# jcyk/gtos

Hardware: AMD Instinct MI355X
Metric: graphs/sec training step (100-node AMR, batch 64) (higher is better)
Workload: dtype bf16

## Files before the change

gtos_amd/build.py:

```python
import os
import subprocess
import sys

CSRC = os.path.join(os.path.dirname(os.path.abspath(__file__)), "csrc")
LIB = os.path.join(CSRC, "libgtos_hip.so")
SOURCES = ["gemm.hip", "rel_attn.hip", "rowops.hip", "gru_step.hip", "copy_nll.hip", "tokenenc.hip", "pathtrie_dev.hip", "relbatch_dev.hip", "relindex_dev.hip", "beam.hip", "sample.hip", "copy_ls.hip", "copy_eval.hip"]
EXACT_FP = {"relbatch_dev.hip", "beam.hip", "sample.hip"}
HIPCC = os.environ.get("HIPCC", "/opt/rocm/bin/hipcc")
FLAGS = ["--offload-arch=gfx950", "-O3", "-std=c++17", "-fPIC", "-ffast-math", "-fno-finite-math-only"]


def _stale(target, deps):
    if not os.path.exists(target):
        return True
    t = os.path.getmtime(target)
    return any(os.path.getmtime(d) > t for d in deps)


def _deps(obj, fallback):
    dfile = obj[:-2] + ".d"
    root = os.path.dirname(os.path.dirname(CSRC))
    try:
        words = open(dfile).read().replace("\\\n", " ").split()
    except OSError:
        return fallback
    deps = [w for w in words[1:] if w.endswith((".h", ".hpp")) and os.path.abspath(w).startswith(root) and os.path.exists(w)]
    return deps or fallback


HOST_SRCS = [os.path.join(os.path.dirname(CSRC), "csrc_host", f) for f in ("relbatch.cpp", "pathtrie.cpp", "relindex.cpp")]
HOST_LIB = os.path.join(os.path.dirname(CSRC), "csrc_host", "libgtos_host.so")
CXX = os.environ.get("CXX", "g++")


def build_host(force=False, verbose=True):
    hdr = os.path.join(os.path.dirname(os.path.dirname(CSRC)), "include", "gtos_host.h")
    shared = [os.path.join(CSRC, h) for h in ("relbatch_kernels.h", "relindex_kernels.h", "trie_kernels.h")]
    if force or _stale(HOST_LIB, HOST_SRCS + [hdr] + shared):
        cmd = [CXX, "-O3", "-std=c++17", "-shared", "-fPIC", "-pthread"] + HOST_SRCS + ["-o", HOST_LIB]
        if verbose:
            print(" ".join(cmd), flush=True)
        subprocess.check_call(cmd)
    return HOST_LIB


def build(force=False, verbose=True):
    build_host(force, verbose)
    own_hdr = {"pathtrie_dev.hip": "trie_kernels.h", "relbatch_dev.hip": "relbatch_kernels.h",
               "relindex_dev.hip": "relindex_kernels.h", "beam.hip": "beam_kernels.h slot_kernels.h slot_device.h",
               "sample.hip": "sample_kernels.h slot_kernels.h slot_device.h", "copy_ls.hip": "copy_ls_kernels.h",
               "copy_nll.hip": "copy_row.h", "copy_eval.hip": "copy_eval_kernels.h"}
    objs = []
    for src in SOURCES:
        s = os.path.join(CSRC, src)
        o = os.path.join(CSRC, src.replace(".hip", ".o"))
        objs.append(o)
        if force or _stale(o, [s] + _deps(o, [os.path.join(CSRC, h) for h in own_hdr.get(src, "common.h").split()])):
            flags = [f for f in FLAGS if f not in ("-ffast-math", "-fno-finite-math-only")] + ["-ffp-contract=off"] if src in EXACT_FP else FLAGS
            cmd = [HIPCC] + flags + ["-MMD", "-MF", o[:-2] + ".d", "-c", s, "-o", o]
            if verbose:
                print(" ".join(cmd), flush=True)
            subprocess.check_call(cmd)
    if force or _stale(LIB, objs):
        cmd = [HIPCC, "--offload-arch=gfx950", "-shared", "-fPIC"] + objs + ["-o", LIB]
        if verbose:
            print(" ".join(cmd), flush=True)
        subprocess.check_call(cmd)
    return LIB


if __name__ == "__main__":
    build(force="--force" in sys.argv)
    print(LIB)
```

gtos_amd/csrc/common.h:

```cpp
#pragma once
#include <hip/hip_runtime.h>
#include <stdint.h>

#define GTOS_F32 0
#define GTOS_BF16 1

typedef uint16_t bf16_t;
typedef __attribute__((ext_vector_type(8))) __bf16 bf16x8_t;
typedef __attribute__((ext_vector_type(8))) short s16x8_t;
typedef __attribute__((ext_vector_type(4))) float f32x4_t;

typedef __attribute__((ext_vector_type(4))) uint32_t U128;

__device__ __forceinline__ float bf2f(bf16_t v) { return __uint_as_float(((uint32_t)v) << 16); }
typedef __attribute__((ext_vector_type(2))) __bf16 bf16x2_hw_t;
typedef __attribute__((ext_vector_type(2))) float f32x2_hw_t;
__device__ __forceinline__ bf16_t f2bf(float f) { return __builtin_bit_cast(bf16_t, static_cast<__bf16>(f)); }
__device__ __forceinline__ float lo_bf(uint32_t w) { return __uint_as_float(w << 16); }
__device__ __forceinline__ float hi_bf(uint32_t w) { return __uint_as_float(w & 0xffff0000u); }
__device__ __forceinline__ uint32_t pack_bf(float a, float b) {
    const f32x2_hw_t v = {a, b};
    return __builtin_bit_cast(uint32_t, __builtin_convertvector(v, bf16x2_hw_t));
}

template <typename T> struct Vec8;
template <> struct Vec8<float> {
    static __device__ __forceinline__ void load(const float* p, float (&v)[8]) {
        const float4 a = *reinterpret_cast<const float4*>(p), b = *reinterpret_cast<const float4*>(p + 4);
        v[0] = a.x; v[1] = a.y; v[2] = a.z; v[3] = a.w; v[4] = b.x; v[5] = b.y; v[6] = b.z; v[7] = b.w;
    }
    static __device__ __forceinline__ void store(float* p, const float (&v)[8]) {
        *reinterpret_cast<float4*>(p) = make_float4(v[0], v[1], v[2], v[3]);
        *reinterpret_cast<float4*>(p + 4) = make_float4(v[4], v[5], v[6], v[7]);
    }
};
template <> struct Vec8<bf16_t> {
    static __device__ __forceinline__ void load(const bf16_t* p, float (&v)[8]) {
        const uint4 a = *reinterpret_cast<const uint4*>(p);
        v[0] = lo_bf(a.x); v[1] = hi_bf(a.x); v[2] = lo_bf(a.y); v[3] = hi_bf(a.y);
        v[4] = lo_bf(a.z); v[5] = hi_bf(a.z); v[6] = lo_bf(a.w); v[7] = hi_bf(a.w);
    }
    static __device__ __forceinline__ void store(bf16_t* p, const float (&v)[8]) {
        *reinterpret_cast<uint4*>(p) = make_uint4(pack_bf(v[0], v[1]), pack_bf(v[2], v[3]),
                                                  pack_bf(v[4], v[5]), pack_bf(v[6], v[7]));
    }
};

template <typename T> __device__ __forceinline__ float to_f(T v);
template <> __device__ __forceinline__ float to_f<float>(float v) { return v; }
template <> __device__ __forceinline__ float to_f<bf16_t>(bf16_t v) { return bf2f(v); }
template <typename T> __device__ __forceinline__ T from_f(float v);
template <> __device__ __forceinline__ float from_f<float>(float v) { return v; }
template <> __device__ __forceinline__ bf16_t from_f<bf16_t>(float v) { return f2bf(v); }

__device__ __forceinline__ uint32_t mix32(uint32_t h) {
    h ^= h >> 16; h *= 0x7feb352dU; h ^= h >> 15; h *= 0x846ca68bU; h ^= h >> 16;
    return h;
}
__device__ __forceinline__ float rand01(uint64_t seed, uint64_t idx) {
    uint32_t h = mix32((uint32_t)idx ^ (uint32_t)seed);
    h = mix32(h + (uint32_t)(idx >> 32) * 0x9E3779B9U + (uint32_t)(seed >> 32));
    return (float)(h >> 8) * (1.0f / 16777216.0f);
}
__device__ __forceinline__ bool drop_keep(uint64_t seed, uint64_t idx, float p) { return rand01(seed, idx) >= p; }

static __device__ const unsigned long long* g_seed_epoch = nullptr;
__device__ __forceinline__ uint64_t live_seed(uint64_t seed) {
    const unsigned long long* p = g_seed_epoch;
    return p ? seed + (uint64_t)(*p) * 0x9E3779B97F4A7C15ull : seed;
}
#define GTOS_SEED_EPOCH_SETTER(tu)                                                                                   \
    extern "C" __attribute__((visibility("hidden"))) int gtosi_##tu##_set_seed_epoch(const void* p) {               \
        return (int)hipMemcpyToSymbol(HIP_SYMBOL(g_seed_epoch), &p, sizeof(p));                                      \
    }
extern "C" __attribute__((visibility("hidden"))) int gtosi_gemm_set_seed_epoch(const void* p);
extern "C" __attribute__((visibility("hidden"))) int gtosi_rel_attn_set_seed_epoch(const void* p);
extern "C" __attribute__((visibility("hidden"))) int gtosi_rowops_set_seed_epoch(const void* p);
extern "C" __attribute__((visibility("hidden"))) int gtosi_gru_step_set_seed_epoch(const void* p);
extern "C" __attribute__((visibility("hidden"))) int gtosi_tokenenc_set_seed_epoch(const void* p);

__device__ __forceinline__ float wave_sum(float v) {
#pragma unroll
    for (int o = 32; o > 0; o >>= 1) v += __shfl_xor(v, o);
    return v;
}
__device__ __forceinline__ float wave_max(float v) {
#pragma unroll
    for (int o = 32; o > 0; o >>= 1) v = fmaxf(v, __shfl_xor(v, o));
    return v;
}

#define GTOS_CHECK_LAUNCH() do { hipError_t e_ = hipGetLastError(); if (e_ != hipSuccess) return (int)e_; } while (0)
```

gtos_amd/csrc/rel_attn.hip:

```cpp
#include "common.h"
#include <cstdlib>
#include <type_traits>

namespace {

template <typename T> struct Raw8;
template <> struct Raw8<bf16_t> {
    uint4 a;
    __device__ __forceinline__ void load(const bf16_t* p) { a = *reinterpret_cast<const uint4*>(p); }
    __device__ __forceinline__ void zero() { a = make_uint4(0, 0, 0, 0); }
    __device__ __forceinline__ void get(float (&v)[8]) const {
        v[0] = lo_bf(a.x); v[1] = hi_bf(a.x); v[2] = lo_bf(a.y); v[3] = hi_bf(a.y);
        v[4] = lo_bf(a.z); v[5] = hi_bf(a.z); v[6] = lo_bf(a.w); v[7] = hi_bf(a.w);
    }
};
template <> struct Raw8<float> {
    float4 a, b;
    __device__ __forceinline__ void load(const float* p) {
        a = *reinterpret_cast<const float4*>(p); b = *reinterpret_cast<const float4*>(p + 4);
    }
    __device__ __forceinline__ void zero() { a = make_float4(0, 0, 0, 0); b = a; }
    __device__ __forceinline__ void get(float (&v)[8]) const {
        v[0] = a.x; v[1] = a.y; v[2] = a.z; v[3] = a.w; v[4] = b.x; v[5] = b.y; v[6] = b.z; v[7] = b.w;
    }
};

#ifndef GTOS_ATTN_U
#define GTOS_ATTN_U 1
#endif
template <typename T> struct Unroll { static constexpr int U = GTOS_ATTN_U; };
template <> struct Unroll<float> { static constexpr int U = 1; };

struct AttnArgs {
    const void *q, *k, *v; int64_t ldq, ldk, ldv;
    const void* rel;
    const int* idx_q;
    const int* idx_k;
    const uint8_t* key_pad;
    const uint8_t* attn_mask;
    void* o; int64_t ldo;
    float* lse;
    float* w;
    const void* d_o; int64_t lddo;
    const float* dw;
    void *dq, *dk, *dv; int64_t lddq, lddk, lddv;
    int64_t ld_drel;
    void* d_rel;
    float* pd;
    float* gs;
    int T, S, B, H, d, mode;
    int hd, nhs, lr;
    float scale, p_drop; uint64_t seed;
};
// ... 494 lines not shown
#pragma unroll
                for (int e = 0; e < 8; ++e) { r1[e] = fmaf(gsum, RB[e], da[e]); r2[e] = fmaf(gsum, RA[e], db[e]); }
                Vec8<T>::store(out, r1);
                Vec8<T>::store(out + d, r2);
            }
        }
        m1 = m2; l1 = l2; m2 = m3;
    }
}

template <typename K> int dispatch_lh(int lh, K&& f) {
    switch (lh) {
        case 1: return f(std::integral_constant<int, 1>());
        case 2: return f(std::integral_constant<int, 2>());
        case 4: return f(std::integral_constant<int, 4>());
        case 8: return f(std::integral_constant<int, 8>());
        case 16: return f(std::integral_constant<int, 16>());
        case 32: return f(std::integral_constant<int, 32>());
        case 64: return f(std::integral_constant<int, 64>());
    }
    return -11;
}

struct Geo { int LH, nhs, lr, slices; bool generic; };
int pow2ceil(int x) { int p = 1; while (p < x) p <<= 1; return p; }
int geometry(int d, int H, Geo& g) {
    if (H <= 0 || d <= 0 || d % H) return -10;
    const int hd = d / H;
    if (hd % 8 || hd > 512) return -10;
    g.generic = !(d <= 512 && (d & (d - 1)) == 0 && (hd & (hd - 1)) == 0);
    if (!g.generic) { g.LH = hd / 8; g.nhs = H; g.lr = d / 8; g.slices = 1; return 0; }
    g.LH = pow2ceil(hd / 8);
    int nhs = 64 / g.LH;
    const int hp = pow2ceil(H);
    if (nhs > hp) nhs = hp;
    g.nhs = nhs; g.lr = nhs * g.LH; g.slices = (H + nhs - 1) / nhs;
    return 0;
}
int check_shape(int d, int H) { Geo g; return geometry(d, H, g); }

int nblocks(int rows, int B) { return rows * B; }

}

static int fill_args(AttnArgs& a, Geo& g, int T_, int S, int B, int H, int d, int mode, float scale, float p_drop, uint64_t seed) {
    a.T = T_; a.S = S; a.B = B; a.H = H; a.d = d; a.mode = mode; a.scale = scale; a.p_drop = p_drop; a.seed = seed;
    if (mode != 0 && T_ != S) return -12;
    const int rc = geometry(d, H, g);
    if (rc) return rc;
    a.hd = d / H; a.nhs = g.nhs; a.lr = g.lr;
    return 0;
}

extern "C" int gtos_rel_attn_fwd(int dtype, int mode, int T_, int S, int B, int H, int d,
                                 const void* q, int64_t ldq, const void* k, int64_t ldk, const void* v, int64_t ldv,
                                 const void* rel, const int* idx_q, const uint8_t* key_pad, const uint8_t* attn_mask,
                                 float scale, float p_drop, uint64_t seed,
                                 void* o, int64_t ldo, float* lse, float* w, void* stream) {
    AttnArgs a = {};
    Geo geo;
    int rc = fill_args(a, geo, T_, S, B, H, d, mode, scale, p_drop, seed);
    if (rc) return rc;
    a.q = q; a.k = k; a.v = v; a.ldq = ldq; a.ldk = ldk; a.ldv = ldv; a.rel = rel; a.idx_q = idx_q;
    a.key_pad = key_pad; a.attn_mask = attn_mask; a.o = o; a.ldo = ldo; a.lse = lse; a.w = w;
    hipStream_t s = static_cast<hipStream_t>(stream);
    const dim3 grid(nblocks(T_, B), geo.slices);
    return dispatch_lh(geo.LH, [&](auto lh) {
        constexpr int LH = decltype(lh)::value;
        if (geo.generic) {
            if (dtype == GTOS_BF16) hipLaunchKernelGGL((rel_attn_fwd_kernel<bf16_t, LH, true>), grid, dim3(256), 0, s, a);
            else hipLaunchKernelGGL((rel_attn_fwd_kernel<float, LH, true>), grid, dim3(256), 0, s, a);
        } else {
            if (dtype == GTOS_BF16) hipLaunchKernelGGL((rel_attn_fwd_kernel<bf16_t, LH, false>), grid, dim3(256), 0, s, a);
            else hipLaunchKernelGGL((rel_attn_fwd_kernel<float, LH, false>), grid, dim3(256), 0, s, a);
        }
        GTOS_CHECK_LAUNCH();
        return 0;
    });
}

extern "C" int gtos_rel_attn_bwd(int dtype, int mode, int T_, int S, int B, int H, int d,
                                 const void* q, int64_t ldq, const void* k, int64_t ldk, const void* v, int64_t ldv,
                                 const void* rel, const int* idx_q, const int* idx_k,
                                 const uint8_t* key_pad, const uint8_t* attn_mask,
                                 float scale, float p_drop, uint64_t seed,
                                 const void* o, int64_t ldo, const float* lse, const float* w,
                                 const void* d_o, int64_t lddo, const float* dw,
                                 void* dq, int64_t lddq, void* dk, int64_t lddk, void* dv, int64_t lddv,
                                 void* d_rel, int64_t ld_drel, float* pd, float* gs, void* stream) {
    AttnArgs a = {};
    Geo geo;
    int rc = fill_args(a, geo, T_, S, B, H, d, mode, scale, p_drop, seed);
    if (rc) return rc;
    a.q = q; a.k = k; a.v = v; a.ldq = ldq; a.ldk = ldk; a.ldv = ldv; a.rel = rel; a.idx_q = idx_q; a.idx_k = idx_k;
    a.key_pad = key_pad; a.attn_mask = attn_mask; a.o = const_cast<void*>(o); a.ldo = ldo;
    a.lse = const_cast<float*>(lse); a.w = const_cast<float*>(w); a.d_o = d_o; a.lddo = lddo; a.dw = dw;
    a.dq = dq; a.dk = dk; a.dv = dv; a.lddq = lddq; a.lddk = lddk; a.lddv = lddv; a.d_rel = d_rel; a.ld_drel = ld_drel; a.pd = pd; a.gs = gs;
    if (mode == 2 && d_rel && (ld_drel < 2 * d || ld_drel % 8)) return -14;
    if (dw && !w) return -13;
    hipStream_t s = static_cast<hipStream_t>(stream);
    const dim3 gq(nblocks(T_, B), geo.slices), gk(nblocks(S, B), geo.slices);
    return dispatch_lh(geo.LH, [&](auto lh) {
        constexpr int LH = decltype(lh)::value;
#define GTOS_BWD(TT, GG) do { hipLaunchKernelGGL((rel_attn_bwd_q_kernel<TT, LH, GG>), gq, dim3(256), 0, s, a); \
                              hipLaunchKernelGGL((rel_attn_bwd_kv_kernel<TT, LH, GG>), gk, dim3(256), 0, s, a); } while (0)
        if (geo.generic) { if (dtype == GTOS_BF16) GTOS_BWD(bf16_t, true); else GTOS_BWD(float, true); }
        else { if (dtype == GTOS_BF16) GTOS_BWD(bf16_t, false); else GTOS_BWD(float, false); }
#undef GTOS_BWD
        GTOS_CHECK_LAUNCH();
        return 0;
    });
}

extern "C" int gtos_rel_attn_bwd_bank(int dtype, int n, int B, int H, int d,
                                      const void* q, int64_t ldq, const void* k, int64_t ldk,
                                      const void* bank, const float* gs,
                                      const int* pair_sorted, const int* chunk_type, const int* chunk_start,
                                      const int* chunk_count, const int* chunk_slot, const int* xcd_off, int nchunks,
                                      void* d_bank, int64_t ld_dbank, float* heavy, void* stream) {
    Geo geo;
    int rc = geometry(d, H, geo);
    if (rc) return rc;
    if (ld_dbank < 2 * d || ld_dbank % 8) return -14;
    if (nchunks <= 0) return 0;
    BankArgs a;
    a.q = q; a.k = k; a.ldq = ldq; a.ldk = ldk; a.bank = bank; a.gs = gs; a.pair_sorted = pair_sorted;
    a.chunk_type = chunk_type; a.chunk_start = chunk_start; a.chunk_count = chunk_count; a.chunk_slot = chunk_slot;
    a.d_bank = d_bank; a.ld_dbank = ld_dbank; a.heavy = heavy; a.nchunks = nchunks; a.T = n; a.S = n; a.B = B; a.H = H; a.d = d;
    a.xcd_off = xcd_off;
    a.hd = d / H; a.nhs = geo.nhs; a.lr = geo.lr;
    hipStream_t s = static_cast<hipStream_t>(stream);
    int grid = (nchunks + 3) / 4; if (grid > 4096) grid = 4096;
    if (xcd_off) grid = (grid + 7) / 8 * 8;
    const dim3 g2(grid, geo.slices);
    return dispatch_lh(geo.LH, [&](auto lh) {
        constexpr int LH = decltype(lh)::value;
        if (geo.generic) {
            if (dtype == GTOS_BF16) hipLaunchKernelGGL((rel_attn_bwd_bank_kernel<bf16_t, LH, true, 4>), g2, dim3(256), 0, s, a);
            else hipLaunchKernelGGL((rel_attn_bwd_bank_kernel<float, LH, true, 4>), g2, dim3(256), 0, s, a);
        } else {
            if (dtype == GTOS_BF16) hipLaunchKernelGGL((rel_attn_bwd_bank_kernel<bf16_t, LH, false, 2>), g2, dim3(256), 0, s, a);
            else hipLaunchKernelGGL((rel_attn_bwd_bank_kernel<float, LH, false, 4>), g2, dim3(256), 0, s, a);
        }
        GTOS_CHECK_LAUNCH();
        return 0;
    });
}

GTOS_SEED_EPOCH_SETTER(rel_attn)
```

gtos_amd/csrc/rowops.hip:

```cpp
#include "common.h"

namespace {

constexpr int LN_MAXC = 2;

template <typename TX, typename TR, typename TY>
__global__ __launch_bounds__(256) void ln_fwd_kernel(int rows, int d, const TX* __restrict__ x, const TR* __restrict__ r,
                                                     float p_drop, uint64_t seed, const float* __restrict__ gamma,
                                                     const float* __restrict__ beta, float eps, TY* __restrict__ y, bf16_t* __restrict__ y2,
                                                     float* __restrict__ mean, float* __restrict__ rstd) {
    if (p_drop > 0.f) seed = live_seed(seed);
    const int lane = threadIdx.x & 63;
    const int row = blockIdx.x * 4 + (threadIdx.x >> 6);
    if (row >= rows) return;
    const float ks = p_drop > 0.f ? 1.f / (1.f - p_drop) : 1.f;
    float z[LN_MAXC][8];
    float s = 0.f;
#pragma unroll
    for (int cI = 0; cI < LN_MAXC; ++cI) {
        const int c = (cI * 64 + lane) * 8;
#pragma unroll
        for (int e = 0; e < 8; ++e) z[cI][e] = 0.f;
        if (c < d) {
            Vec8<TX>::load(x + (int64_t)row * d + c, z[cI]);
// ... 1060 lines not shown
extern "C" int gtos_adam_step(int64_t n, float* p, const float* g, float* m, float* v, float lr, float beta1, float beta2,
                              float eps, float weight_decay, float gscale, const float* sqnorm, float max_norm,
                              void* bf16_mirror, void* stream) {
    if (n <= 0) return 0;
    hipStream_t s = static_cast<hipStream_t>(stream);
    hipLaunchKernelGGL(adam_kernel, dim3(grid_for(n, 256 * 4)), dim3(256), 0, s, n, p, g, m, v, lr, beta1, beta2, eps, weight_decay,
                       gscale, sqnorm, max_norm, (bf16_t*)bf16_mirror, (const float*)nullptr);
    GTOS_CHECK_LAUNCH();
    return 0;
}

extern "C" int gtos_adam_step_ctl(int64_t n, float* p, const float* g, float* m, float* v, const float* ctl, float beta1, float beta2,
                                  float eps, float weight_decay, float gscale, const float* sqnorm, float max_norm,
                                  void* bf16_mirror, void* stream) {
    if (n <= 0) return 0;
    if (!ctl) return -23;
    hipStream_t s = static_cast<hipStream_t>(stream);
    hipLaunchKernelGGL(adam_kernel, dim3(grid_for(n, 256 * 4)), dim3(256), 0, s, n, p, g, m, v, 0.f, beta1, beta2, eps, weight_decay,
                       gscale, sqnorm, max_norm, (bf16_t*)bf16_mirror, ctl);
    GTOS_CHECK_LAUNCH();
    return 0;
}

extern "C" int gtos_step_control(int phase, const float* loss, double* state, float* flag, int warmup_steps, int embed_dim,
                                 float* ctl, void* stream) {
    if ((phase != 0 && phase != 1) || !loss || !state || !flag || !ctl || warmup_steps < 1 || embed_dim < 1) return -23;
    hipLaunchKernelGGL(step_control_kernel, dim3(1), dim3(64), 0, static_cast<hipStream_t>(stream), phase, loss, state, flag,
                       (double)warmup_steps, (double)embed_dim, ctl);
    GTOS_CHECK_LAUNCH();
    return 0;
}

extern "C" int gtos_cast_f32_to_bf16(int64_t n, const float* src, void* dst, void* stream) {
    if (n <= 0) return 0;
    hipStream_t s = static_cast<hipStream_t>(stream);
    hipLaunchKernelGGL(cast_bf16_kernel, dim3(grid_for(n, 256 * 4)), dim3(256), 0, s, n, src, (bf16_t*)dst);
    GTOS_CHECK_LAUNCH();
    return 0;
}

extern "C" int gtos_transpose_batch_bf16(int n_mat, const int64_t* desc, const int* tile_start, int total_tiles, const void* src,
                                         void* dst, void* stream) {
    if (n_mat <= 0 || total_tiles <= 0) return 0;
    if (!desc || !tile_start || !src || !dst) return -23;
    hipLaunchKernelGGL(transpose_batch_kernel, dim3((unsigned)total_tiles), dim3(256), 0, static_cast<hipStream_t>(stream), n_mat, desc,
                       tile_start, (const bf16_t*)src, (bf16_t*)dst);
    GTOS_CHECK_LAUNCH();
    return 0;
}

extern "C" int gtos_set_seed_epoch(const void* epoch) {
    int rc = gtosi_gemm_set_seed_epoch(epoch);
    if (!rc) rc = gtosi_rel_attn_set_seed_epoch(epoch);
    if (!rc) rc = gtosi_rowops_set_seed_epoch(epoch);
    if (!rc) rc = gtosi_gru_step_set_seed_epoch(epoch);
    if (!rc) rc = gtosi_tokenenc_set_seed_epoch(epoch);
    return rc;
}

extern "C" int gtos_abi_version(void) { return 25; }

GTOS_SEED_EPOCH_SETTER(rowops)
```

gtos_amd/ops.py:

```python
import contextlib
import os

import torch

from . import _lib
from ._lib import call, dt, ptr, require_cuda, stream

_seed_state = [0x5DEECE66D]

PROFILE = None
PROFILE_DETAIL = False
GEMM_PROFILE = None


class _Timed:

    def __init__(self, name, detail=False, units=0):
        self.name, self.units = name, units
        self.on = PROFILE is not None and (PROFILE_DETAIL or not detail)

    def __enter__(self):
        if self.on:
            self.s = torch.cuda.Event(enable_timing=True)
            self.e = torch.cuda.Event(enable_timing=True)
# ... 625 lines not shown
        starts = bounds[:-1]
        nch = torch.clamp((counts + self.CHUNK - 1) // self.CHUNK, min=1)
        ctype = torch.repeat_interleave(torch.arange(R, device=flat.device), nch)
        first = torch.cumsum(nch, 0) - nch
        local = torch.arange(ctype.numel(), device=flat.device) - first[ctype]
        heavy_types = torch.nonzero(nch > 1).flatten()
        slot_of_type = torch.full((R,), -1, dtype=torch.int64, device=flat.device)
        slot_of_type[heavy_types] = torch.arange(heavy_types.numel(), device=flat.device)
        self.pair_sorted = order.to(torch.int32)
        c_type = ctype.to(torch.int32)
        c_start = (starts[ctype] + local * self.CHUNK).to(torch.int32)
        c_count = torch.clamp(counts[ctype] - local * self.CHUNK, min=0, max=self.CHUNK).to(torch.int32)
        c_slot = slot_of_type[ctype].to(torch.int32)
        first = self.pair_sorted[c_start.clamp(max=flat.numel() - 1).long()]
        gb = first % B
        xcd = (gb // (B // 8)) if B % 8 == 0 else (gb % 8)
        xs, perm = torch.sort(xcd.to(torch.int32), stable=True)
        self.xcd_off = torch.searchsorted(xs, torch.arange(9, device=flat.device, dtype=torch.int32)).to(torch.int32)
        self.chunk_type, self.chunk_start = c_type[perm], c_start[perm]
        self.chunk_count, self.chunk_slot = c_count[perm], c_slot[perm]
        self.heavy_types = heavy_types.to(torch.int32)
        self.nchunks = int(ctype.numel())

    def prefetch_projections(self, attns):
        self._proj = {}
        if not (PROJ_SIDE and self.bank.is_cuda and side_ok(self.bank.device) and torch.is_grad_enabled()):
            return
        dev = self.bank.device
        main, side = torch.cuda.current_stream(dev), side_stream(dev)
        if any(m.compute_dtype != self.bank.dtype for m in attns):
            return
        if sum(self.bank.shape[0] * m.relation_in_proj.weight.shape[0] for m in attns) * self.bank.element_size() > PROJ_SIDE_MAX_BYTES:
            return
        side.wait_stream(main)
        self.bank.record_stream(side)
        with torch.cuda.stream(side):
            for m in attns:
                y = linear(self.bank, m.relation_in_proj.weight, group=self.grad_group)
                ev = torch.cuda.Event()
                ev.record(side)
                self._proj[id(m)] = (y, ev)

    def take_projection(self, attn):
        hit = self._proj.pop(id(attn), None)
        if hit is None:
            return None
        y, ev = hit
        main = torch.cuda.current_stream(y.device)
        main.wait_event(ev)
        y.record_stream(main)
        return y


class RelAttnFn(torch.autograd.Function):

    @staticmethod
    def forward(ctx, qsrc, kvsrc, rel, fact, offs, d, H, scale, key_pad, attn_mask, p_drop, need_w):
        require_cuda(qsrc, kvsrc, rel)
        q_off, k_off, v_off = offs
        kv = qsrc if kvsrc is None else kvsrc
        assert qsrc.is_contiguous() and kv.is_contiguous()
        T_, B, Cq = qsrc.shape
        S, _, Ckv = kv.shape
        mode = 0 if rel is None else (2 if fact is not None else 1)
        if mode == 1:
            assert rel.is_contiguous() and tuple(rel.shape) == (S, T_, B, 2 * d)
        o = torch.empty((T_, B, d), dtype=qsrc.dtype, device=qsrc.device)
        lse = torch.empty((T_, B, H), dtype=torch.float32, device=qsrc.device)
        w = torch.empty((T_, S, B, H), dtype=torch.float32, device=qsrc.device) if need_w else None
        seed = next_seed() if p_drop > 0 else 0
        es = qsrc.element_size()
        with _Timed("rel_attn_fwd_mode%d" % mode):
            call("gtos_rel_attn_fwd", dt(qsrc), mode, T_, S, B, H, d,
                 qsrc.data_ptr() + q_off * es, Cq, kv.data_ptr() + k_off * es, Ckv, kv.data_ptr() + v_off * es, Ckv,
                 ptr(rel), ptr(fact.idx_q) if fact is not None else None, ptr(key_pad), ptr(attn_mask),
                 float(scale), float(p_drop), seed, ptr(o), d, ptr(lse), ptr(w), stream())
        src = getattr(rel, "_gtos_proj_src", None) if (mode == 2 and PROJ_RECOMPUTE) else None
        ctx.save_for_backward(qsrc, kvsrc, rel if src is None else None, o, lse, w, key_pad, attn_mask)
        ctx.cfg = (fact, offs, d, H, scale, p_drop, seed, mode)
        ctx.proj_src = src
        return o, w

    @staticmethod
    def backward(ctx, d_o, d_w):
        qsrc, kvsrc, rel, o, lse, w, key_pad, attn_mask = ctx.saved_tensors
        fact, (q_off, k_off, v_off), d, H, scale, p_drop, seed, mode = ctx.cfg
        if ctx.proj_src is not None:
            bank_, w_ = ctx.proj_src
            rel = gemm(bank_, w_, trans_b=True)
        kv = qsrc if kvsrc is None else kvsrc
        T_, B, Cq = qsrc.shape
        S, _, Ckv = kv.shape
        d_o = d_o.contiguous()
        if d_w is not None:
            d_w = d_w.contiguous().float()
        full_q = (Cq == d) if kvsrc is not None else (Cq == 3 * d)
        dqsrc = (torch.empty_like if full_q else torch.zeros_like)(qsrc)
        dkv = dqsrc if kvsrc is None else (torch.empty_like if Ckv == 2 * d else torch.zeros_like)(kvsrc)
        if mode == 1:
            d_rel = torch.empty_like(rel)
        elif mode == 2:
            d_rel = fact.grad_group.grad_slice(rel) if ctx.needs_input_grad[2] else None
            if d_rel is None:
                d_rel = torch.empty_like(rel)
        else:
            d_rel = None
        ldr = d_rel.stride(0) if mode == 2 else 0
        pd = torch.empty((T_, S, B, H), dtype=torch.float32, device=qsrc.device)
        gs = torch.empty_like(pd)
        es = qsrc.element_size()
        with _Timed("rel_attn_bwd_q+kv_mode%d" % mode, detail=True):
            call("gtos_rel_attn_bwd", dt(qsrc), mode, T_, S, B, H, d,
                 qsrc.data_ptr() + q_off * es, Cq, kv.data_ptr() + k_off * es, Ckv, kv.data_ptr() + v_off * es, Ckv,
                 ptr(rel), ptr(fact.idx_q) if fact is not None else None, ptr(fact.idx_k) if fact is not None else None,
                 ptr(key_pad), ptr(attn_mask), float(scale), float(p_drop), seed,
                 ptr(o), d, ptr(lse), ptr(w), ptr(d_o), d, ptr(d_w),
                 dqsrc.data_ptr() + q_off * es, Cq, dkv.data_ptr() + k_off * es, Ckv, dkv.data_ptr() + v_off * es, Ckv,
                 ptr(d_rel), ldr, ptr(pd), ptr(gs), stream())
        if mode == 2:
            nh = int(fact.heavy_types.numel())
            heavy = torch.zeros((max(nh, 1), 2 * d), dtype=torch.float32, device=rel.device)
            with _Timed("rel_attn_bwd_bank", detail=True):
                call("gtos_rel_attn_bwd_bank", dt(qsrc), T_, B, H, d,
                     qsrc.data_ptr() + q_off * es, Cq, kv.data_ptr() + k_off * es, Ckv,
                     ptr(rel), ptr(gs), ptr(fact.pair_sorted), ptr(fact.chunk_type), ptr(fact.chunk_start),
                     ptr(fact.chunk_count), ptr(fact.chunk_slot), ptr(fact.xcd_off), fact.nchunks, ptr(d_rel), ldr, ptr(heavy), stream())
            if nh and d_rel.dtype == torch.bfloat16:
                call("gtos_segment_sum_finish", nh, ptr(fact.heavy_types), ptr(heavy), 2 * d, ptr(d_rel), ldr, stream())
            elif nh:
                d_rel[fact.heavy_types.long()] = heavy[:nh].to(d_rel.dtype)
        return dqsrc, (dkv if kvsrc is not None else None), d_rel, None, None, None, None, None, None, None, None, None


def attention_core(qsrc, kvsrc, offs, d, H, scale, rel=None, fact=None, key_pad=None, attn_mask=None,
                   p_drop=0.0, need_weights=False):
    return RelAttnFn.apply(qsrc, kvsrc, rel, fact, offs, d, H, scale, _u8(key_pad), _u8(attn_mask),
                           float(p_drop), need_weights)


def factored_eval_relation(bank, relation):
    n, n2, B, K = relation.shape
    tuples, inv = torch.unique(relation.reshape(-1, K), dim=0, return_inverse=True)
    bank_c = relation_gather_mean(bank, tuples, zero_row0=True)
    return FactoredRelation(bank_c, inv.view(n, n2, B))


def relation_gather_mean(bank, idx, zero_row0):
    require_cuda(bank, idx)
    K = idx.shape[-1] if zero_row0 else 1
    lead = idx.shape[:-1] if zero_row0 else idx.shape
    P = idx.numel() // K
    bank = bank.contiguous()
    out = torch.empty((P, bank.shape[1]), dtype=bank.dtype, device=bank.device)
    call("gtos_relation_gather_mean", dt(bank), P, K, bank.shape[1], ptr(bank), ptr(idx.contiguous()), int(zero_row0),
         ptr(out), stream())
    return out.view(*lead, bank.shape[1])


def embed_bwd_workspace(n, V, dim_pad, device):
    if V * dim_pad * 4 > 60 * 1024 or n <= 8 * 512:
        return None
    return torch.empty((min(2048, (n + 511) // 512), V * dim_pad), dtype=torch.float32, device=device)

# ... 370 lines not shown
```

Baseline: 852.1.

## Add MFMA flash-style tiled attention kernels for plain bf16 attention mode

Adds a new tiled attention forward and backward path, used for mode 0 (no relation bias) bf16 attention when head dims are 32/64/128. It stages K/V tiles in shared memory and computes scores and outputs with MFMA bf16 instructions and an online softmax, with a hi/lo split of the probabilities to keep precision. The backward pass runs dK/dV and dQ blocks in one fused launch and no longer allocates the full T×S×B×H fp32 pd/gs scratch tensors. Risks include numeric differences from the old path, and it only applies to mode 0 calls with aligned pointers.

```diff
diff --git a/gtos_amd/build.py b/gtos_amd/build.py
--- a/gtos_amd/build.py
+++ b/gtos_amd/build.py
@@ -4,7 +4,7 @@
 
 CSRC = os.path.join(os.path.dirname(os.path.abspath(__file__)), "csrc")
 LIB = os.path.join(CSRC, "libgtos_hip.so")
-SOURCES = ["gemm.hip", "rel_attn.hip", "rowops.hip", "gru_step.hip", "copy_nll.hip", "tokenenc.hip", "pathtrie_dev.hip", "relbatch_dev.hip", "relindex_dev.hip", "beam.hip", "sample.hip", "copy_ls.hip", "copy_eval.hip"]
+SOURCES = ["gemm.hip", "rel_attn.hip", "attn_tile.hip", "rowops.hip", "gru_step.hip", "copy_nll.hip", "tokenenc.hip", "pathtrie_dev.hip", "relbatch_dev.hip", "relindex_dev.hip", "beam.hip", "sample.hip", "copy_ls.hip", "copy_eval.hip"]
 EXACT_FP = {"relbatch_dev.hip", "beam.hip", "sample.hip"}
 HIPCC = os.environ.get("HIPCC", "/opt/rocm/bin/hipcc")
 FLAGS = ["--offload-arch=gfx950", "-O3", "-std=c++17", "-fPIC", "-ffast-math", "-fno-finite-math-only"]
@@ -49,7 +49,8 @@
     own_hdr = {"pathtrie_dev.hip": "trie_kernels.h", "relbatch_dev.hip": "relbatch_kernels.h",
                "relindex_dev.hip": "relindex_kernels.h", "beam.hip": "beam_kernels.h slot_kernels.h slot_device.h",
                "sample.hip": "sample_kernels.h slot_kernels.h slot_device.h", "copy_ls.hip": "copy_ls_kernels.h",
-               "copy_nll.hip": "copy_row.h", "copy_eval.hip": "copy_eval_kernels.h"}
+               "copy_nll.hip": "copy_row.h", "rel_attn.hip": "common.h attn_tile.h", "attn_tile.hip": "common.h attn_tile.h",
+               "copy_eval.hip": "copy_eval_kernels.h"}
     objs = []
     for src in SOURCES:
         s = os.path.join(CSRC, src)
diff --git a/gtos_amd/csrc/attn_tile.h b/gtos_amd/csrc/attn_tile.h
--- /dev/null
+++ b/gtos_amd/csrc/attn_tile.h
@@ -0,0 +1,20 @@
+#pragma once
+#include <stdint.h>
+
+struct AttnTileArgs {
+    const void *q, *k, *v; int64_t ldq, ldk, ldv;
+    const uint8_t* key_pad;
+    const uint8_t* attn_mask;
+    void* o; int64_t ldo;
+    float* lse;
+    float* w;
+    const void* d_o; int64_t lddo;
+    const float* dw;
+    void *dq, *dk, *dv; int64_t lddq, lddk, lddv;
+    int T, S, B, H, d;
+    float scale, p_drop; uint64_t seed;
+};
+
+bool gtosi_attn_tile_covers(int T, int S, int B, int H, int d, const AttnTileArgs& a, bool backward);
+int gtosi_attn_tile_fwd(const AttnTileArgs& a, void* stream);
+int gtosi_attn_tile_bwd(const AttnTileArgs& a, void* stream);
diff --git a/gtos_amd/csrc/attn_tile.hip b/gtos_amd/csrc/attn_tile.hip
--- /dev/null
+++ b/gtos_amd/csrc/attn_tile.hip
@@ -0,0 +1,422 @@
+#include "common.h"
+#include "attn_tile.h"
+#include <cstdlib>
+#include <type_traits>
+
+namespace {
+
+constexpr int OWN = 64;
+
+template <int HD> struct Cfg {
+    static constexpr int NT = HD == 128 ? 32 : 64;
+    static constexpr int RS = HD + 8;
+    static constexpr int CH = HD / 8;
+    static constexpr int KC = HD / 32;
+    static constexpr int CB = HD / 16;
+    static constexpr int NB = NT / 32;
+    static constexpr int DS = NT + 4;
+};
+
+__device__ __forceinline__ void map_block(int B, int H, int& b, int& h, int& tile) {
+    const int blk = blockIdx.x;
+    int rest;
+    if ((B & 7) == 0) { const int x = blk & 7, w = blk >> 3, gpx = B >> 3; b = x * gpx + (w % gpx); rest = w / gpx; }
+    else { b = blk % B; rest = blk / B; }
+    h = rest % H; tile = rest / H;
+}
+
+__device__ __forceinline__ f32x4_t mfma(bf16x8_t a, bf16x8_t b, f32x4_t c) {
+    return __builtin_amdgcn_mfma_f32_16x16x32_bf16(a, b, c, 0, 0, 0);
+}
+
+template <int HD, bool RM, bool TR>
+__device__ __forceinline__ void stage(const bf16_t* __restrict__ base, int64_t rstride, int r0, int nrows, bf16_t* rm, bf16_t* tr) {
+    using C = Cfg<HD>;
+    constexpr int IT = C::NT * C::CH / 256;
+    uint4 v[IT];
+#pragma unroll
+    for (int it = 0; it < IT; ++it) {
+        const int idx = it * 256 + threadIdx.x, y = idx / C::CH, c = idx % C::CH;
+        v[it] = make_uint4(0, 0, 0, 0);
+        if (r0 + y < nrows) v[it] = *reinterpret_cast<const uint4*>(base + (int64_t)(r0 + y) * rstride + c * 8);
+    }
+#pragma unroll
+    for (int it = 0; it < IT; ++it) {
+        const int idx = it * 256 + threadIdx.x, y = idx / C::CH, c = idx % C::CH;
+        if (RM) *reinterpret_cast<uint4*>(rm + y * C::RS + c * 8) = v[it];
+        if (TR) {
+            const int yc = (((y >> 3) ^ (c & (C::NT / 8 - 1))) << 3) | (y & 7);
+            const uint32_t ww[4] = {v[it].x, v[it].y, v[it].z, v[it].w};
+#pragma unroll
+            for (int e = 0; e < 8; ++e) tr[(c * 8 + e) * C::NT + yc] = (bf16_t)(ww[e >> 1] >> ((e & 1) * 16));
+        }
+    }
+}
+
+template <int HD> __device__ __forceinline__ bf16x8_t frag_rows(const bf16_t* rm, int kb, int t, int kc, int lane) {
+    const int r = lane & 15, row = kb * 32 + (r >> 2) * 8 + t * 4 + (r & 3);
+    return *reinterpret_cast<const bf16x8_t*>(rm + row * Cfg<HD>::RS + kc * 32 + (lane >> 4) * 8);
+}
+template <int HD> __device__ __forceinline__ bf16x8_t frag_tr(const bf16_t* tr, int cb, int kb, int lane) {
+    constexpr int NT = Cfg<HD>::NT;
+    const int cc = cb * 16 + (lane & 15), chunk = (kb * 4 + (lane >> 4)) ^ ((cc >> 3) & (NT / 8 - 1));
+    return *reinterpret_cast<const bf16x8_t*>(tr + cc * NT + chunk * 8);
+}
+template <int HD> __device__ __forceinline__ void load_own(const bf16_t* __restrict__ base, int64_t rstride, int x, bool valid, int lane,
+                                                            bf16x8_t (&f)[Cfg<HD>::KC]) {
+#pragma unroll
+    for (int kc = 0; kc < Cfg<HD>::KC; ++kc) {
+        U128 v = {0, 0, 0, 0};
+        if (valid) v = *reinterpret_cast<const U128*>(base + (int64_t)x * rstride + kc * 32 + (lane >> 4) * 8);
+        f[kc] = __builtin_bit_cast(bf16x8_t, v);
+    }
+}
+__device__ __forceinline__ void split8(const float (&p)[8], bf16x8_t& hi, bf16x8_t& lo) {
+    uint32_t hw[4], lw[4];
+#pragma unroll
+    for (int e = 0; e < 4; ++e) {
+        hw[e] = pack_bf(p[2 * e], p[2 * e + 1]);
+        lw[e] = pack_bf(p[2 * e] - lo_bf(hw[e]), p[2 * e + 1] - hi_bf(hw[e]));
+    }
+    const U128 a = {hw[0], hw[1], hw[2], hw[3]}, b = {lw[0], lw[1], lw[2], lw[3]};
+    hi = __builtin_bit_cast(bf16x8_t, a); lo = __builtin_bit_cast(bf16x8_t, b);
+}
+__device__ __forceinline__ void store4(bf16_t* p, const f32x4_t& v, float s) {
+    *reinterpret_cast<uint2*>(p) = make_uint2(pack_bf(v[0] * s, v[1] * s), pack_bf(v[2] * s, v[3] * s));
+}
+
+template <int HD, bool KM>
+__device__ __forceinline__ void fill_dead(const AttnTileArgs& a, int b, int x0, int y0, unsigned char* sdead) {
+    using C = Cfg<HD>;
+#pragma unroll
+    for (int it = 0; it < OWN * C::NT / 256; ++it) {
+        const int idx = it * 256 + threadIdx.x, xo = idx / C::NT, ys = idx % C::NT;
+        const int i = KM ? y0 + ys : x0 + xo, j = KM ? x0 + xo : y0 + ys;
+        const int ic = min(i, a.T - 1), jc = min(j, a.S - 1);
+        const unsigned char kp = a.key_pad ? a.key_pad[(int64_t)jc * a.B + b] : 0;
+        const unsigned char am = a.attn_mask ? a.attn_mask[(int64_t)ic * a.S + jc] : 0;
+        sdead[xo * C::DS + ys] = (i >= a.T || j >= a.S || kp != 0 || am != 0) ? 1 : 0;
+    }
+}
+
+template <int HD>
+__global__ __launch_bounds__(256) void attn_tile_fwd_kernel(AttnTileArgs a) {
+    using C = Cfg<HD>;
+    if (a.p_drop > 0.f) a.seed = live_seed(a.seed);
+    __shared__ __attribute__((aligned(16))) bf16_t sK[C::NT * C::RS];
+    __shared__ __attribute__((aligned(16))) bf16_t sVt[HD * C::NT];
+    __shared__ __attribute__((aligned(16))) unsigned char sdead[OWN * C::DS];
+    int b, h, qt;
+    map_block(a.B, a.H, b, h, qt);
+    const int lane = threadIdx.x & 63, wv = threadIdx.x >> 6, n = lane & 15, g = lane >> 4;
+    const int i0 = qt * OWN, xo = wv * 16 + n, i = i0 + xo;
+    const bool iv = i < a.T;
+    const int64_t hb = (int64_t)h * HD;
+    const bf16_t* qb = static_cast<const bf16_t*>(a.q) + (int64_t)b * a.ldq + hb;
+    const bf16_t* kb_ = static_cast<const bf16_t*>(a.k) + (int64_t)b * a.ldk + hb;
+    const bf16_t* vb = static_cast<const bf16_t*>(a.v) + (int64_t)b * a.ldv + hb;
+    const int64_t rsq = (int64_t)a.B * a.ldq, rsk = (int64_t)a.B * a.ldk, rsv = (int64_t)a.B * a.ldv;
+    const float keep_scale = a.p_drop > 0.f ? 1.f / (1.f - a.p_drop) : 1.f;
+
+    bf16x8_t xq[C::KC];
+    load_own<HD>(qb, rsq, i, iv, lane, xq);
+    float m = -INFINITY, l = 0.f;
+    f32x4_t oacc[C::CB];
+#pragma unroll
+    for (int cb = 0; cb < C::CB; ++cb) oacc[cb] = f32x4_t{0.f, 0.f, 0.f, 0.f};
+
+    for (int j0 = 0; j0 < a.S; j0 += C::NT) {
+        __syncthreads();
+        stage<HD, true, false>(kb_, rsk, j0, a.S, sK, nullptr);
+        stage<HD, false, true>(vb, rsv, j0, a.S, nullptr, sVt);
+        fill_dead<HD, false>(a, b, i0, j0, sdead);
+        __syncthreads();
+        float s[C::NB][8];
+        float mt = -INFINITY;
+#pragma unroll
+        for (int kb = 0; kb < C::NB; ++kb) {
+#pragma unroll
+            for (int t = 0; t < 2; ++t) {
+                f32x4_t part[C::KC];
+#pragma unroll
+                for (int kc = 0; kc < C::KC; ++kc) part[kc] = mfma(frag_rows<HD>(sK, kb, t, kc, lane), xq[kc], f32x4_t{0.f, 0.f, 0.f, 0.f});
+                f32x4_t acc = part[0];
+                if (C::KC == 2) acc = part[0] + part[1];
+                if (C::KC == 4) acc = (part[0] + part[1]) + (part[2] + part[3]);
+                const uint32_t dd = *reinterpret_cast<const uint32_t*>(sdead + xo * C::DS + kb * 32 + g * 8 + t * 4);
+#pragma unroll
+                for (int e = 0; e < 4; ++e) {
+                    const bool dead = ((dd >> (8 * e)) & 0xff) != 0;
+                    const float sv = dead ? -INFINITY : acc[e] * a.scale;
+                    s[kb][t * 4 + e] = sv;
+                    mt = fmaxf(mt, sv);
+                    const int j = j0 + kb * 32 + g * 8 + t * 4 + e;
+                    if (a.w && iv && j < a.S) a.w[(((int64_t)i * a.S + j) * a.B + b) * a.H + h] = sv;
+                }
+            }
+        }
+        mt = fmaxf(mt, __shfl_xor(mt, 16));
+        mt = fmaxf(mt, __shfl_xor(mt, 32));
+        const float mn = fmaxf(m, mt);
+        float alpha = 1.f, lsum = 0.f;
+        if (mn != -INFINITY) alpha = __expf(m - mn);
+#pragma unroll
+        for (int kb = 0; kb < C::NB; ++kb) {
+#pragma unroll
+            for (int e = 0; e < 8; ++e) {
+                const float sv = s[kb][e];
+                float pe = 0.f;
+                if (mn != -INFINITY) pe = __expf(sv - mn);
+                lsum += pe;
+                if (a.p_drop > 0.f && sv != -INFINITY) {
+                    const int j = j0 + kb * 32 + g * 8 + e;
+                    pe = drop_keep(a.seed, (((uint64_t)i * a.S + j) * a.B + b) * a.H + h, a.p_drop) ? pe * keep_scale : 0.f;
+                }
+                s[kb][e] = pe;
+            }
+        }
+        lsum += __shfl_xor(lsum, 16);
+        lsum += __shfl_xor(lsum, 32);
+        l = l * alpha + lsum;
+        m = mn;
+#pragma unroll
+        for (int cb = 0; cb < C::CB; ++cb) oacc[cb] *= alpha;
+#pragma unroll
+        for (int kb = 0; kb < C::NB; ++kb) {
+            bf16x8_t ph, pl;
+            split8(s[kb], ph, pl);
+#pragma unroll
+            for (int cb = 0; cb < C::CB; ++cb) {
+                const bf16x8_t vt = frag_tr<HD>(sVt, cb, kb, lane);
+                oacc[cb] = mfma(vt, ph, oacc[cb]);
+                oacc[cb] = mfma(vt, pl, oacc[cb]);
+            }
+        }
+    }
+    const float inv = l > 0.f ? 1.f / l : 0.f;
+    if (iv) {
+        bf16_t* op = static_cast<bf16_t*>(a.o) + ((int64_t)i * a.B + b) * a.ldo + hb + g * 4;
+#pragma unroll
+        for (int cb = 0; cb < C::CB; ++cb) store4(op + cb * 16, oacc[cb], inv);
+        if (g == 0) a.lse[((int64_t)i * a.B + b) * a.H + h] = (l > 0.f) ? m + __logf(l) : -INFINITY;
+    }
+    if (a.w && iv) {
+        for (int jb = g * 8; jb < a.S; jb += 32) {
+            for (int e = 0; e < 8 && jb + e < a.S; ++e) {
+                const int64_t off = (((int64_t)i * a.S + jb + e) * a.B + b) * a.H + h;
+                const float sv = a.w[off];
+                float p = (sv == -INFINITY || inv <= 0.f) ? 0.f : __expf(sv - m) * inv;
+                if (a.p_drop > 0.f && p > 0.f) p = drop_keep(a.seed, (uint64_t)off, a.p_drop) ? p * keep_scale : 0.f;
+                a.w[off] = p;
+            }
+        }
+    }
+}
+
+template <int HD>
+__device__ __forceinline__ void row_stats(const AttnTileArgs& a, int b, int h, int i0, int cnt, float* sLse, float* sD) {
+    const int row = threadIdx.x >> 2, part = threadIdx.x & 3, i = i0 + row;
+    const bool valid = row < cnt && i < a.T;
+    float acc = 0.f;
+    if (valid) {
+        const int64_t hb = (int64_t)h * HD + part * (HD / 4);
+        const bf16_t* dop = static_cast<const bf16_t*>(a.d_o) + ((int64_t)i * a.B + b) * a.lddo + hb;
+        const bf16_t* op = static_cast<const bf16_t*>(a.o) + ((int64_t)i * a.B + b) * a.ldo + hb;
+#pragma unroll
+        for (int c = 0; c < HD / 32; ++c) {
+            float x[8], y[8];
+            Vec8<bf16_t>::load(dop + c * 8, x);
+            Vec8<bf16_t>::load(op + c * 8, y);
+#pragma unroll
+            for (int e = 0; e < 8; ++e) acc = fmaf(x[e], y[e], acc);
+        }
+        if (a.dw) {
+            for (int j = part; j < a.S; j += 4) {
+                const int64_t off = (((int64_t)i * a.S + j) * a.B + b) * a.H + h;
+                acc = fmaf(a.w[off], a.dw[off], acc);
+            }
+        }
+    }
+    acc += __shfl_xor(acc, 1);
+    acc += __shfl_xor(acc, 2);
+    if (part == 0 && row < cnt) {
+        sD[row] = acc;
+        sLse[row] = valid ? a.lse[((int64_t)i * a.B + b) * a.H + h] : -INFINITY;
+    }
+}
+
+struct BwdSmem { bf16_t *y1, *y2, *y1t, *y2t; unsigned char* dead; float *lse, *dl; };
+
+template <int HD, bool KM>
+__device__ __forceinline__ void bwd_body(const AttnTileArgs& a, int b, int h, int tile, const BwdSmem& sm) {
+    using C = Cfg<HD>;
+    const int lane = threadIdx.x & 63, wv = threadIdx.x >> 6, n = lane & 15, g = lane >> 4;
+    const int nX = KM ? a.S : a.T, nY = KM ? a.T : a.S;
+    const int x0 = tile * OWN, xo = wv * 16 + n, x = x0 + xo;
+    const bool xv = x < nX;
+    const int64_t hb = (int64_t)h * HD;
+    const bf16_t* qb = static_cast<const bf16_t*>(a.q) + (int64_t)b * a.ldq + hb;
+    const bf16_t* kb_ = static_cast<const bf16_t*>(a.k) + (int64_t)b * a.ldk + hb;
+    const bf16_t* vb = static_cast<const bf16_t*>(a.v) + (int64_t)b * a.ldv + hb;
+    const bf16_t* dob = static_cast<const bf16_t*>(a.d_o) + (int64_t)b * a.lddo + hb;
+    const int64_t rsq = (int64_t)a.B * a.ldq, rsk = (int64_t)a.B * a.ldk, rsv = (int64_t)a.B * a.ldv, rsdo = (int64_t)a.B * a.lddo;
+    const float keep_scale = a.p_drop > 0.f ? 1.f / (1.f - a.p_drop) : 1.f;
+
+    bf16x8_t x1[C::KC], x2[C::KC];
+    if (KM) { load_own<HD>(kb_, rsk, x, xv, lane, x1); load_own<HD>(vb, rsv, x, xv, lane, x2); }
+    else { load_own<HD>(qb, rsq, x, xv, lane, x1); load_own<HD>(dob, rsdo, x, xv, lane, x2); }
+    f32x4_t acc1[C::CB], acc2[KM ? C::CB : 1];
+#pragma unroll
+    for (int cb = 0; cb < C::CB; ++cb) { acc1[cb] = f32x4_t{0.f, 0.f, 0.f, 0.f}; if (KM) acc2[cb] = f32x4_t{0.f, 0.f, 0.f, 0.f}; }
+    float lse_own = -INFINITY, d_own = 0.f;
+    if (!KM) {
+        row_stats<HD>(a, b, h, x0, OWN, sm.lse, sm.dl);
+        __syncthreads();
+        lse_own = sm.lse[xo]; d_own = sm.dl[xo];
+    }
+    for (int y0 = 0; y0 < nY; y0 += C::NT) {
+        __syncthreads();
+        if (KM) {
+            stage<HD, true, true>(qb, rsq, y0, a.T, sm.y1, sm.y1t);
+            stage<HD, true, true>(dob, rsdo, y0, a.T, sm.y2, sm.y2t);
+            row_stats<HD>(a, b, h, y0, C::NT, sm.lse, sm.dl);
+        } else {
+            stage<HD, true, true>(kb_, rsk, y0, a.S, sm.y1, sm.y1t);
+            stage<HD, true, false>(vb, rsv, y0, a.S, sm.y2, nullptr);
+        }
+        fill_dead<HD, KM>(a, b, x0, y0, sm.dead);
+        __syncthreads();
+#pragma unroll
+        for (int kb = 0; kb < C::NB; ++kb) {
+            float pd[8], gs[8];
+#pragma unroll
+            for (int t = 0; t < 2; ++t) {
+                f32x4_t sa = {0.f, 0.f, 0.f, 0.f}, da = {0.f, 0.f, 0.f, 0.f};
+#pragma unroll
+                for (int kc = 0; kc < C::KC; ++kc) {
+                    sa = mfma(frag_rows<HD>(sm.y1, kb, t, kc, lane), x1[kc], sa);
+                    da = mfma(frag_rows<HD>(sm.y2, kb, t, kc, lane), x2[kc], da);
+                }
+                const int ys = kb * 32 + g * 8 + t * 4;
+                const uint32_t dd = *reinterpret_cast<const uint32_t*>(sm.dead + xo * C::DS + ys);
+#pragma unroll
+                for (int e = 0; e < 4; ++e) {
+                    const int y = y0 + ys + e;
+                    const int i = KM ? y : x, j = KM ? x : y;
+                    const float lse = KM ? sm.lse[ys + e] : lse_own, dl = KM ? sm.dl[ys + e] : d_own;
+                    const bool dead = ((dd >> (8 * e)) & 0xff) != 0 || lse == -INFINITY;
+                    const float p = dead ? 0.f : __expf(sa[e] * a.scale - lse);
+                    const bool inr = i < a.T && j < a.S;
+                    const int64_t off = (((int64_t)i * a.S + j) * a.B + b) * a.H + h;
+                    float keep = 1.f;
+                    if (a.p_drop > 0.f) keep = drop_keep(a.seed, (uint64_t)off, a.p_drop) ? keep_scale : 0.f;
+                    float dp = da[e];
+                    if (a.dw && inr) dp += a.dw[off];
+                    pd[t * 4 + e] = p * keep;
+                    gs[t * 4 + e] = a.scale * p * (keep * dp - dl);
+                }
+            }
+            bf16x8_t gh, gl;
+            split8(gs, gh, gl);
+#pragma unroll
+            for (int cb = 0; cb < C::CB; ++cb) {
+                const bf16x8_t yt = frag_tr<HD>(sm.y1t, cb, kb, lane);
+                acc1[cb] = mfma(yt, gh, acc1[cb]);
+                acc1[cb] = mfma(yt, gl, acc1[cb]);
+            }
+            if (KM) {
+                bf16x8_t ph, pl;
+                split8(pd, ph, pl);
+#pragma unroll
+                for (int cb = 0; cb < C::CB; ++cb) {
+                    const bf16x8_t yt = frag_tr<HD>(sm.y2t, cb, kb, lane);
+                    acc2[cb] = mfma(yt, ph, acc2[cb]);
+                    acc2[cb] = mfma(yt, pl, acc2[cb]);
+                }
+            }
+        }
+    }
+    if (xv) {
+        if (KM) {
+            bf16_t* dkp = static_cast<bf16_t*>(a.dk) + ((int64_t)x * a.B + b) * a.lddk + hb + g * 4;
+            bf16_t* dvp = static_cast<bf16_t*>(a.dv) + ((int64_t)x * a.B + b) * a.lddv + hb + g * 4;
+#pragma unroll
+            for (int cb = 0; cb < C::CB; ++cb) { store4(dkp + cb * 16, acc1[cb], 1.f); store4(dvp + cb * 16, acc2[cb], 1.f); }
+        } else {
+            bf16_t* dqp = static_cast<bf16_t*>(a.dq) + ((int64_t)x * a.B + b) * a.lddq + hb + g * 4;
+#pragma unroll
+            for (int cb = 0; cb < C::CB; ++cb) store4(dqp + cb * 16, acc1[cb], 1.f);
+        }
+    }
+}
+
+template <int HD>
+__global__ __launch_bounds__(256) void attn_tile_bwd_kernel(AttnTileArgs a, int nkt) {
+    using C = Cfg<HD>;
+    if (a.p_drop > 0.f) a.seed = live_seed(a.seed);
+    __shared__ __attribute__((aligned(16))) bf16_t sY1[C::NT * C::RS];
+    __shared__ __attribute__((aligned(16))) bf16_t sY2[C::NT * C::RS];
+    __shared__ __attribute__((aligned(16))) bf16_t sY1t[HD * C::NT];
+    __shared__ __attribute__((aligned(16))) bf16_t sY2t[HD * C::NT];
+    __shared__ __attribute__((aligned(16))) unsigned char sdead[OWN * C::DS];
+    __shared__ __attribute__((aligned(16))) float sLse[OWN];
+    __shared__ __attribute__((aligned(16))) float sDl[OWN];
+    const BwdSmem sm = {sY1, sY2, sY1t, sY2t, sdead, sLse, sDl};
+    int b, h, tile;
+    map_block(a.B, a.H, b, h, tile);
+    if (tile < nkt) bwd_body<HD, true>(a, b, h, tile, sm);
+    else bwd_body<HD, false>(a, b, h, tile - nkt, sm);
+}
+
+bool aligned(const void* p, int n) { return (reinterpret_cast<uintptr_t>(p) & (uintptr_t)(n - 1)) == 0; }
+
+template <typename K> int dispatch_hd(int hd, K&& f) {
+    switch (hd) {
+        case 32: return f(std::integral_constant<int, 32>());
+        case 64: return f(std::integral_constant<int, 64>());
+        case 128: return f(std::integral_constant<int, 128>());
+    }
+    return -11;
+}
+
+}
+
+bool gtosi_attn_tile_covers(int T_, int S, int B, int H, int d, const AttnTileArgs& a, bool backward) {
+    const char* sw = getenv("GTOS_ATTN_TILE");
+    if (sw && sw[0] == '0') return false;
+    if (T_ < 16 || S < 1 || B < 1 || H < 1 || d > 512 || (d & (d - 1)) || d % H) return false;
+    const int hd = d / H;
+    if (hd != 32 && hd != 64 && hd != 128) return false;
+    if (a.ldq % 8 || a.ldk % 8 || a.ldv % 8 || a.ldo % 4 || !aligned(a.q, 16) || !aligned(a.k, 16) || !aligned(a.v, 16) || !aligned(a.o, 16))
+        return false;
+    if (backward && (a.lddo % 8 || a.ldo % 8 || a.lddq % 4 || a.lddk % 4 || a.lddv % 4 || !aligned(a.d_o, 16) || !aligned(a.dq, 8) ||
+                     !aligned(a.dk, 8) || !aligned(a.dv, 8)))
+        return false;
+    return true;
+}
+
+int gtosi_attn_tile_fwd(const AttnTileArgs& a, void* stream) {
+    hipStream_t s = static_cast<hipStream_t>(stream);
+    const int nqt = (a.T + OWN - 1) / OWN;
+    const dim3 grid(a.B * a.H * nqt);
+    return dispatch_hd(a.d / a.H, [&](auto hd) {
+        constexpr int HD = decltype(hd)::value;
+        hipLaunchKernelGGL((attn_tile_fwd_kernel<HD>), grid, dim3(256), 0, s, a);
+        GTOS_CHECK_LAUNCH();
+        return 0;
+    });
+}
+
+int gtosi_attn_tile_bwd(const AttnTileArgs& a, void* stream) {
+    hipStream_t s = static_cast<hipStream_t>(stream);
+    const int nqt = (a.T + OWN - 1) / OWN, nkt = (a.S + OWN - 1) / OWN;
+    const dim3 grid(a.B * a.H * (nqt + nkt));
+    return dispatch_hd(a.d / a.H, [&](auto hd) {
+        constexpr int HD = decltype(hd)::value;
+        hipLaunchKernelGGL((attn_tile_bwd_kernel<HD>), grid, dim3(256), 0, s, a, nkt);
+        GTOS_CHECK_LAUNCH();
+        return 0;
+    });
+}
+
+GTOS_SEED_EPOCH_SETTER(attn_tile)
diff --git a/gtos_amd/csrc/common.h b/gtos_amd/csrc/common.h
--- a/gtos_amd/csrc/common.h
+++ b/gtos_amd/csrc/common.h
@@ -75,6 +75,7 @@
     }
 extern "C" __attribute__((visibility("hidden"))) int gtosi_gemm_set_seed_epoch(const void* p);
 extern "C" __attribute__((visibility("hidden"))) int gtosi_rel_attn_set_seed_epoch(const void* p);
+extern "C" __attribute__((visibility("hidden"))) int gtosi_attn_tile_set_seed_epoch(const void* p);
 extern "C" __attribute__((visibility("hidden"))) int gtosi_rowops_set_seed_epoch(const void* p);
 extern "C" __attribute__((visibility("hidden"))) int gtosi_gru_step_set_seed_epoch(const void* p);
 extern "C" __attribute__((visibility("hidden"))) int gtosi_tokenenc_set_seed_epoch(const void* p);
diff --git a/gtos_amd/csrc/rel_attn.hip b/gtos_amd/csrc/rel_attn.hip
--- a/gtos_amd/csrc/rel_attn.hip
+++ b/gtos_amd/csrc/rel_attn.hip
@@ -1,4 +1,5 @@
 #include "common.h"
+#include "attn_tile.h"
 #include <cstdlib>
 #include <type_traits>
 
@@ -599,6 +600,15 @@
     return 0;
 }
 
+static AttnTileArgs tile_args(const AttnArgs& a) {
+    AttnTileArgs t = {};
+    t.q = a.q; t.k = a.k; t.v = a.v; t.ldq = a.ldq; t.ldk = a.ldk; t.ldv = a.ldv; t.key_pad = a.key_pad; t.attn_mask = a.attn_mask;
+    t.o = a.o; t.ldo = a.ldo; t.lse = a.lse; t.w = a.w; t.d_o = a.d_o; t.lddo = a.lddo; t.dw = a.dw;
+    t.dq = a.dq; t.dk = a.dk; t.dv = a.dv; t.lddq = a.lddq; t.lddk = a.lddk; t.lddv = a.lddv;
+    t.T = a.T; t.S = a.S; t.B = a.B; t.H = a.H; t.d = a.d; t.scale = a.scale; t.p_drop = a.p_drop; t.seed = a.seed;
+    return t;
+}
+
 extern "C" int gtos_rel_attn_fwd(int dtype, int mode, int T_, int S, int B, int H, int d,
                                  const void* q, int64_t ldq, const void* k, int64_t ldk, const void* v, int64_t ldv,
                                  const void* rel, const int* idx_q, const uint8_t* key_pad, const uint8_t* attn_mask,
@@ -610,6 +620,10 @@
     if (rc) return rc;
     a.q = q; a.k = k; a.v = v; a.ldq = ldq; a.ldk = ldk; a.ldv = ldv; a.rel = rel; a.idx_q = idx_q;
     a.key_pad = key_pad; a.attn_mask = attn_mask; a.o = o; a.ldo = ldo; a.lse = lse; a.w = w;
+    if (mode == 0 && dtype == GTOS_BF16 && !geo.generic) {
+        const AttnTileArgs t = tile_args(a);
+        if (gtosi_attn_tile_covers(T_, S, B, H, d, t, false)) return gtosi_attn_tile_fwd(t, stream);
+    }
     hipStream_t s = static_cast<hipStream_t>(stream);
     const dim3 grid(nblocks(T_, B), geo.slices);
     return dispatch_lh(geo.LH, [&](auto lh) {
@@ -645,6 +659,11 @@
     a.dq = dq; a.dk = dk; a.dv = dv; a.lddq = lddq; a.lddk = lddk; a.lddv = lddv; a.d_rel = d_rel; a.ld_drel = ld_drel; a.pd = pd; a.gs = gs;
     if (mode == 2 && d_rel && (ld_drel < 2 * d || ld_drel % 8)) return -14;
     if (dw && !w) return -13;
+    if (mode == 0 && dtype == GTOS_BF16 && !geo.generic) {
+        const AttnTileArgs t = tile_args(a);
+        if (gtosi_attn_tile_covers(T_, S, B, H, d, t, true)) return gtosi_attn_tile_bwd(t, stream);
+    }
+    if (!pd || !gs) return -15;
     hipStream_t s = static_cast<hipStream_t>(stream);
     const dim3 gq(nblocks(T_, B), geo.slices), gk(nblocks(S, B), geo.slices);
     return dispatch_lh(geo.LH, [&](auto lh) {
diff --git a/gtos_amd/csrc/rowops.hip b/gtos_amd/csrc/rowops.hip
--- a/gtos_amd/csrc/rowops.hip
+++ b/gtos_amd/csrc/rowops.hip
@@ -1136,6 +1136,7 @@
 extern "C" int gtos_set_seed_epoch(const void* epoch) {
     int rc = gtosi_gemm_set_seed_epoch(epoch);
     if (!rc) rc = gtosi_rel_attn_set_seed_epoch(epoch);
+    if (!rc) rc = gtosi_attn_tile_set_seed_epoch(epoch);
     if (!rc) rc = gtosi_rowops_set_seed_epoch(epoch);
     if (!rc) rc = gtosi_gru_step_set_seed_epoch(epoch);
     if (!rc) rc = gtosi_tokenenc_set_seed_epoch(epoch);
diff --git a/gtos_amd/ops.py b/gtos_amd/ops.py
--- a/gtos_amd/ops.py
+++ b/gtos_amd/ops.py
@@ -701,6 +701,14 @@
         return y
 
 
+def _attn_tile_backward(mode, T_, d, H, lds, tensors):
+    if mode != 0 or os.environ.get("GTOS_ATTN_TILE", "1")[:1] == "0":
+        return False
+    if any(t.dtype != torch.bfloat16 or t.data_ptr() % 16 for t in tensors) or any(ld % 8 for ld in lds):
+        return False
+    return T_ >= 16 and d <= 512 and d & (d - 1) == 0 and d % H == 0 and d // H in (32, 64, 128)
+
+
 class RelAttnFn(torch.autograd.Function):
 
     @staticmethod
@@ -755,9 +763,12 @@
         else:
             d_rel = None
         ldr = d_rel.stride(0) if mode == 2 else 0
-        pd = torch.empty((T_, S, B, H), dtype=torch.float32, device=qsrc.device)
-        gs = torch.empty_like(pd)
         es = qsrc.element_size()
+        if _attn_tile_backward(mode, T_, d, H, (Cq, Ckv, d, q_off, k_off, v_off), (qsrc, kv, o, d_o, dqsrc, dkv)):
+            pd = gs = None
+        else:
+            pd = torch.empty((T_, S, B, H), dtype=torch.float32, device=qsrc.device)
+            gs = torch.empty_like(pd)
         with _Timed("rel_attn_bwd_q+kv_mode%d" % mode, detail=True):
             call("gtos_rel_attn_bwd", dt(qsrc), mode, T_, S, B, H, d,
                  qsrc.data_ptr() + q_off * es, Cq, kv.data_ptr() + k_off * es, Ckv, kv.data_ptr() + v_off * es, Ckv,
```

Result: faster. 864.3, median of 6 (+1.4%).
